# SKA-INAF/caesar-yolo

Measured on AMD Instinct MI355X. Metric: 512x512 tiles/sec over 16k x 16k FITS, higher is better.
Workload: dtype f16

## Files before the change

caesar_yolo_amd/csrc/conv_igemm.hip:

```cpp
#include "cy_kernels.h"
#include <cmath>
#include <cstdlib>
#include <cstring>
#include <vector>

namespace cy {

typedef _Float16 f16;
typedef f16 f16x8 __attribute__((ext_vector_type(8)));
typedef f16 f16x4 __attribute__((ext_vector_type(4)));
typedef float f32x4 __attribute__((ext_vector_type(4)));
typedef unsigned int u32x4 __attribute__((ext_vector_type(4)));
typedef unsigned int u32x2 __attribute__((ext_vector_type(2)));

#define CY_OOB 0xFFFFFF00u
#define CY_WAIT_VM(N) asm volatile("s_waitcnt vmcnt(%0)" ::"n"(N) : "memory")

#ifndef CY_STAMPS_ENABLED
#define CY_STAMPS_ENABLED 0
#endif
__device__ unsigned long long g_stamps[8];
constexpr int WG_STAMP_SLOTS = 4096;
__device__ unsigned long long g_wg_stamps[WG_STAMP_SLOTS * 4];
__device__ __forceinline__ unsigned long long stamp_now() {
// ... 2500 lines not shown
        }
    }
    if (stamps && tid == 0) {
        unsigned long long* rec = g_wg_stamps + (size_t)(blockIdx.x % WG_STAMP_SLOTS) * 4;
        rec[0] = t_loop - t_entry; rec[1] = t_epi - t_loop; rec[2] = stamp_real() - t_epi; rec[3] = c_epi - c_loop;
    }
}

template <int NB, int MI, int RING, bool K3, bool SPLIT = false, int NDW = 8, bool FUSE2 = false>
static hipError_t launch_direct(const ConvArgs& a, hipStream_t s) {
    constexpr int BN = 64 * NB, BM = 8 * MI * 16;
    const size_t lds = (FUSE2 ? 4 : RING) * BN * 128 + 2048;
    static bool attr_set = false;
    if (!attr_set) {
        hipFuncSetAttribute(reinterpret_cast<const void*>(conv1x1_direct_kernel<NB, MI, RING, K3, SPLIT, NDW, FUSE2>), hipFuncAttributeMaxDynamicSharedMemorySize, (int)lds);
        attr_set = true;
    }
    const int M = a.B * a.Ho * a.Wo;
    const int blocks = ((M + BM - 1) / BM) * ((pad64(a.Cout) + BN - 1) / BN);
    hipLaunchKernelGGL((conv1x1_direct_kernel<NB, MI, RING, K3, SPLIT, NDW, FUSE2>), dim3(blocks), dim3(512), lds, s, a);
    return hipGetLastError();
}

template <int WM, int RING>
static hipError_t launch_halo(const ConvArgs& a, hipStream_t s) {
    constexpr int TH = 4 * WM, NT = WM * 128;
    constexpr int PR = (TH + 2) * 18, NWI = (PR + 7) / 8, NW = NT / 64, PROUNDS = (NWI + NW - 1) / NW;
    const size_t lds = 2 * PROUNDS * NW * 1024 + RING * 128 * 128;
    static bool attr_set = false;
    if (!attr_set) {
        hipFuncSetAttribute(reinterpret_cast<const void*>(conv3x3_halo_kernel<WM, RING>), hipFuncAttributeMaxDynamicSharedMemorySize, (int)lds);
        attr_set = true;
    }
    const int blocks = a.B * ((a.Hi + TH - 1) / TH) * ((a.Wi + 15) / 16) * ((pad64(a.Cout) + 127) / 128);
    hipLaunchKernelGGL((conv3x3_halo_kernel<WM, RING>), dim3(blocks), dim3(NT), lds, s, a);
    return hipGetLastError();
}

template <typename T, int WM, int WN, int MI, int NSTAGE = 2, bool SPLIT = false>
static hipError_t launch_t(const ConvArgs& a, hipStream_t s) {
    constexpr int BM = WM * MI * 16, BN = WN * 64;
    const int M = a.B * a.Ho * a.Wo;
    const int ntm = (M + BM - 1) / BM, ntn = (pad64(a.Cout) + BN - 1) / BN;
    const size_t lds = NSTAGE * (BM + BN) * 128;
    static bool attr_set = false;
    if (!attr_set) {
// ... 44 lines not shown
    const size_t lds = head_pair_lds(p, a, b);
    static bool attr_set = false;
    if (!attr_set) {
        hipFuncSetAttribute(reinterpret_cast<const void*>(head1x1_pair_kernel<false>), hipFuncAttributeMaxDynamicSharedMemorySize, 128 * 1024);
        hipFuncSetAttribute(reinterpret_cast<const void*>(head1x1_pair_kernel<true>), hipFuncAttributeMaxDynamicSharedMemorySize, 128 * 1024);
        attr_set = true;
    }
    const long M = (long)a.B * a.Ho * a.Wo;
    const long wgs = (M + 255) / 256;
    const unsigned grid = (unsigned)(wgs < 256 ? wgs : 256);
    if (p == PREC_F16X3) hipLaunchKernelGGL((head1x1_pair_kernel<true>), dim3(grid), dim3(512), lds, s, a, b, head_rows(b), head_pair_pitch(a.out_ct));
    else hipLaunchKernelGGL((head1x1_pair_kernel<false>), dim3(grid), dim3(512), lds, s, a, b, head_rows(b), head_pair_pitch(a.out_ct));
    return hipGetLastError();
}

static const char* const kVariantNames[CONV_NUM_VARIANTS] = {
    "conv_igemm_kernel<2,2,4> generic 128x128", "conv_igemm_kernel<4,1,2> generic 128x64",
    "conv3x3_halo2_kernel 3x3 s1 16x16px x128ch (halo<2,2> for odd slab counts)", "conv3x3_pp_kernel<2> 3x3 s1 16x16px x64ch",
    "conv3x3_c64_kernel<64|32> 3x3 s1 persistent, Cin 64 or 32", "conv_igemm_kernel<4,2,4,3> generic 256x128, 3-slab ring",
    "conv3x3_wide_kernel 3x3 s1 16x32px x128ch, K slabs of 32",
    "conv1x1_direct_kernel<4,2> 1x1 256px x256ch, pixels to regs", "conv1x1_direct_kernel<2,2> 1x1 256px x128ch, pixels to regs",
    "conv3x3_wide_kernel<WN=1> 3x3 s1 16x32px x64ch", "conv3x3_wide_kernel<dual> 3x3 s1 2 images x 16x16px x128ch",
    "conv3x3_widep_kernel<strip> 3x3 s1 512 flattened px x128ch, persistent",
    "head1x1_kernel detect-head output 1x1, weights stationary in LDS, fp32 rows"};
const char* conv_variant_name(int v) { return v >= 0 && v < CONV_NUM_VARIANTS ? kVariantNames[v] : "?"; }

bool batch_invariant() { const char* e = getenv("CY_BATCH_INVARIANT"); return !e || atoi(e) != 0; }

static int conv_variant_x3(const ConvArgs& a) {
    const bool narrow = pad64(a.Cout) <= 64;
    if (a.k == 3 && a.s == 1 && a.c1 == 0 && !a.up0 && !a.out_f32 && a.Cin % 64 == 0 && a.wgt32 && a.out_bs == a.Ho * a.Wo && a.out_ro == 0) {
        const int wpad = (a.Wi + 31) / 32 * 32;
        const bool fits = (wpad - a.Wi) * 8 <= a.Wi;
        if (narrow && a.Wi % 32 == 0) return CONV_WIDE_64;
        if (narrow && a.Cin >= 128 && env_knob("CY_STRIP", 1) && strip_small(a) && strip_fits(a)) return CONV_STRIP_128;
        if (!narrow && env_knob("CY_STRIP", 1) && strip_fits(a) && strip_cover(a.Hi, a.Wi) + 0.04 < wide2d_cover(a.Hi, a.Wi)) return CONV_STRIP_128;
        if (!narrow && fits) return CONV_WIDE_128;
        if (!narrow && a.Wi <= 16 && a.Wi >= 14) return CONV_WIDE_DUAL;
    }
    if (!a.out_f32 && a.Cin % 64 == 0 && !narrow &&
        ((a.k == 1 && a.s == 1 && (a.c1 == 0 || a.c0 % 64 == 0)) || (a.k == 3 && a.s == 2 && a.c1 == 0 && !a.up0)))
        return pad64(a.Cout) >= 256 ? CONV_DIRECT_256 : CONV_DIRECT_128;
    if (head_direct(a, a.split)) return CONV_HEAD_1X1;
    return narrow ? CONV_GENERIC_64 : CONV_GENERIC_128;
}

int conv_variant(Precision p, const ConvArgs& a) {
    if (p == PREC_F16X3) return conv_variant_x3(a);
    const bool narrow = pad64(a.Cout) <= 64;
    const long Bv = batch_invariant() && a.B < 256 ? 256 : a.B;
    if (p == PREC_F16 && a.k == 3 && a.s == 1 && a.c1 == 0 && !a.up0 && !a.out_f32 && a.Cin == 32 && narrow && a.wgt32 &&
        a.out_bs == a.Ho * a.Wo && a.out_ro == 0)
        return CONV_C64_PERSIST;
    if (p == PREC_F16 && a.k == 3 && a.s == 1 && a.c1 == 0 && !a.up0 && !a.out_f32 && a.Cin % 64 == 0 &&
        a.out_bs == a.Ho * a.Wo && a.out_ro == 0) {
        if (narrow && a.wgt32 && a.Cin >= 128 && a.Wi % 32 == 0 && Bv * ((a.Hi + 15) / 16) * (a.Wi / 32) >= 256) return CONV_WIDE_64;
        if (narrow && a.wgt32 && a.Cin >= 128 && env_knob("CY_STRIP", 1) && strip_small(a) && strip_fits(a)) return CONV_STRIP_128;
        if (narrow && a.Cin == 64) return CONV_C64_PERSIST;
        if (narrow) return CONV_PP_64;
        const int strip = env_knob("CY_STRIP", 1);
        if (strip && a.wgt32 && strip_fits(a) && strip_cover(a.Hi, a.Wi) + 0.04 < wide2d_cover(a.Hi, a.Wi) &&
            (strip > 1 || strip_small(a) || Bv * (long)(a.Hi + 1) * (a.Wi + 1) / 512 * ((pad64(a.Cout) + 127) / 128) >= 200))
            return CONV_STRIP_128;
        const int wpad = (a.Wi + 31) / 32 * 32;
        if (a.wgt32 && (wpad - a.Wi) * 8 <= a.Wi) return CONV_WIDE_128;
        const int dual = getenv("CY_WIDE_DUAL") ? atoi(getenv("CY_WIDE_DUAL")) : 1;
        if (dual && a.wgt32 && a.Wi <= 16 && a.Wi >= 14 &&
            ((Bv + 1) / 2) * ((a.Hi + 15) / 16) * ((pad64(a.Cout) + 127) / 128) >= (dual > 1 ? 1 : 224))
            return CONV_WIDE_DUAL;
        return CONV_HALO8_128;
    }
    if (p == PREC_F16 && head_direct(a, 1)) return CONV_HEAD_1X1;
    if (narrow) return CONV_GENERIC_64;
    if (p == PREC_F16 && !a.out_f32 && a.Cin % 64 == 0 &&
        ((a.k == 1 && a.s == 1 && (a.c1 == 0 || a.c0 % 64 == 0)) || (a.k == 3 && a.s == 2 && a.c1 == 0 && !a.up0 && (a.Cin >= 128 || pad64(a.Cout) < 256)))) {
        const char* e = getenv("CY_DIRECT_MIN_BLOCKS");
        const long min_blocks = e ? atol(e) : 256;
        const int bn = pad64(a.Cout) >= 256 ? 256 : 128;
        const long blocks = ((Bv * a.Ho * a.Wo + 255) / 256) * ((pad64(a.Cout) + bn - 1) / bn);
        if (min_blocks >= 0 && blocks >= min_blocks) return bn == 256 ? CONV_DIRECT_256 : CONV_DIRECT_128;
    }
    const long M = Bv * a.Ho * a.Wo;
    if (p == PREC_F16 && (M / 256) * ((pad64(a.Cout) + 127) / 128) >= 256) return CONV_GENERIC_BIG;
    return CONV_GENERIC_128;
}

hipError_t launch_conv(Precision p, const ConvArgs& a, hipStream_t s) {
    if (p == PREC_F16X3) {
        if ((a.split != 2 && a.split != 3) || !a.oscale) return hipErrorInvalidValue;
        switch (conv_variant_x3(a)) {
            case CONV_WIDE_128:
                if (env_knob("CY_X3_PERSIST", 0) && a.Cout % 16 == 0) return launch_widep(a, s);
                return launch_wide<2, false, true>(a, s);
            case CONV_STRIP_128: return launch_strip(a, s);
            case CONV_WIDE_64: return launch_wide<1, false, true>(a, s);
            case CONV_WIDE_DUAL: return launch_wide<2, true, true>(a, s);
            case CONV_DIRECT_256: return a.k == 3 ? launch_direct<4, 2, 3, true, true>(a, s) : launch_direct<4, 2, 3, false, true>(a, s);
            case CONV_DIRECT_128: return a.k == 3 ? launch_direct<2, 4, 2, true, true>(a, s) : launch_direct<2, 2, 2, false, true>(a, s);
            case CONV_HEAD_1X1: return launch_head<true>(a, s);
            case CONV_GENERIC_64: return launch_t<f16, 4, 1, 2, 2, true>(a, s);
            default: return launch_t<f16, 2, 2, 4, 2, true>(a, s);
        }
    }
// ... 4 lines not shown
            ConvArgs b2 = a; b2.dbg = dev_knob("CY_DBG", 0);
            if ((a.Cin / 64) % 2 == 0) return launch_halo2(b2, s);
            return launch_halo<2, 2>(b2, s);
        }
        case CONV_GENERIC_BIG: return launch_t<f16, 4, 2, 4, 3>(a, s);
        case CONV_WIDE_128: {
            ConvArgs b2 = a; b2.dbg = dev_knob("CY_DBG", 0);
            const int wp = env_knob("CY_WIDE_PERSIST", 1);
            const long patches = (long)a.B * ((a.Wi + 31) / 32) * ((a.Hi + 15) / 16) * ((pad64(a.Cout) + 127) / 128);
            if (wp && a.Cout % 16 == 0 && (wp > 1 || (patches >= 512 && a.Cin <= 128))) return launch_widep(b2, s);
            return launch_wide<2>(b2, s);
        }
        case CONV_STRIP_128: return launch_strip(a, s);
        case CONV_WIDE_64: return launch_wide<1>(a, s);
        case CONV_WIDE_DUAL: return launch_wide<2, true>(a, s);
        case CONV_DIRECT_256: {
            ConvArgs a2 = a; a2.dbg = dev_knob("CY_DBG", 0);
            if (a.wgt2 && pad64(a.Cout) == 256 && a.c1 == 0 && !a.res && !a.out_f32)
                return a.k == 3 ? launch_direct<4, 2, 3, true, false, 4, true>(a2, s) : launch_direct<4, 2, 3, false, false, 8, true>(a2, s);
            return a.k == 3 ? launch_direct<4, 2, 3, true, false, 4>(a2, s) : launch_direct<4, 2, 3, false>(a2, s);
        }
        case CONV_DIRECT_128:
            return a.k == 3 ? launch_direct<2, 4, 2, true>(a, s) : launch_direct<2, 2, 2, false>(a, s);
        case CONV_HEAD_1X1: return launch_head<false>(a, s);
        case CONV_GENERIC_64: return p == PREC_F16 ? launch_t<f16, 4, 1, 2>(a, s) : launch_t<float, 4, 1, 2>(a, s);
        default: return p == PREC_F16 ? launch_t<f16, 2, 2, 4>(a, s) : launch_t<float, 2, 2, 4>(a, s);
    }
}

void debug_read_wg_stamps(unsigned long long* out, int n) {
    hipDeviceSynchronize();
    hipMemcpyFromSymbol(out, HIP_SYMBOL(g_wg_stamps), (size_t)(n < WG_STAMP_SLOTS ? n : WG_STAMP_SLOTS) * 4 * sizeof(unsigned long long));
}

void debug_read_stamps(unsigned long long* out8, bool reset) {
    hipDeviceSynchronize();
    hipMemcpyFromSymbol(out8, HIP_SYMBOL(g_stamps), 8 * sizeof(unsigned long long));
    if (CY_STAMPS_ENABLED && out8[6] == 0) {
        static unsigned long long rec[WG_STAMP_SLOTS * 4];
        hipMemcpyFromSymbol(rec, HIP_SYMBOL(g_wg_stamps), sizeof(rec));
        for (int i = 0; i < WG_STAMP_SLOTS; ++i)
            if (rec[i * 4 + 1]) { out8[6] += 1; for (int j = 0; j < 4; ++j) out8[j] += rec[i * 4 + j]; }
        out8[4] = out8[0] + out8[1] + out8[2] + out8[3];
        if (reset) { memset(rec, 0, sizeof(rec)); hipMemcpyToSymbol(HIP_SYMBOL(g_wg_stamps), rec, sizeof(rec)); }
    }
    if (reset) { unsigned long long z[8] = {0}; hipMemcpyToSymbol(HIP_SYMBOL(g_stamps), z, sizeof(z)); }
// ... 761 lines not shown
```

caesar_yolo_amd/csrc/cy_kernels.h:

```cpp
#pragma once
#include <hip/hip_runtime.h>
#include <stdint.h>
#include <stdlib.h>

namespace cy {

#ifndef CY_DEV_KNOBS
#define CY_DEV_KNOBS 0
#endif
inline int env_knob(const char* name, int dflt) { const char* e = getenv(name); return e ? atoi(e) : dflt; }
inline int dev_knob(const char* name, int dflt) { return CY_DEV_KNOBS ? env_knob(name, dflt) : dflt; }

enum Precision { PREC_F16 = 0, PREC_F32 = 1, PREC_F16X3 = 2 };

struct ConvArgs {
    const void* in0; int in0_ct, in0_coff, c0, up0;
    const void* in1; int in1_ct, in1_coff, c1;
    const void* wgt;
    const void* wgt32; uint32_t wgt32_bytes;
    const float* bias;
    void* out; int out_ct, out_coff;
    int out_bs, out_ro;
    int out_f32;
    const void* res; int res_ct, res_coff;
// ... 34 lines not shown
hipError_t launch_bneck64(const BneckArgs& a, hipStream_t s);
void pack_bneck_weights(const float* W1, const float* W2, void* dst);

struct PoolArgs {
    const void* src; void* dst; int ct, src_coff, dst_coff, C, B, H, W;
    int lo;
};

struct DwArgs {
    const void* in; int in_ct, in_coff; void* out; int out_ct, out_coff; const void* res; int res_ct, res_coff;
    const float* w; const float* bias; int B, H, W, C, act;
    int blk, gstride, goff;
    int in_lo, out_lo, res_lo;
    int xcd;
};
struct AttnArgs {
    const void* qkv; int ct, coff; void* out; int out_ct, out_coff; int B, N, heads, kd, hd; float scale;
    int lo, out_lo;
};
hipError_t launch_dwconv(Precision p, const DwArgs& a, hipStream_t s);
hipError_t launch_attention(Precision p, const AttnArgs& a, hipStream_t s);

hipError_t launch_conv(Precision p, const ConvArgs& a, hipStream_t s);
enum ConvVariant { CONV_GENERIC_128 = 0, CONV_GENERIC_64, CONV_HALO8_128, CONV_PP_64, CONV_C64_PERSIST, CONV_GENERIC_BIG, CONV_WIDE_128, CONV_DIRECT_256, CONV_DIRECT_128, CONV_WIDE_64, CONV_WIDE_DUAL, CONV_STRIP_128, CONV_HEAD_1X1, CONV_NUM_VARIANTS };
int conv_variant(Precision p, const ConvArgs& a);
const char* conv_variant_name(int v);
bool head_pair_ok(Precision p, const ConvArgs& a, const ConvArgs& b);
hipError_t launch_head_pair(Precision p, const ConvArgs& a, const ConvArgs& b, hipStream_t s);
void debug_read_stamps(unsigned long long* out8, bool reset);
void debug_read_wg_stamps(unsigned long long* out, int n);
void debug_read_pre_stamps(unsigned long long* out8, bool reset);
void debug_fastdiv(const double* d_a, const double* d_b, double* d_fast, double* d_ref, int n);
hipError_t launch_stem(Precision p, const StemArgs& a, hipStream_t s);
hipError_t launch_stem_down(const StemDownArgs& a, hipStream_t s);
long stem_down_blocks(const StemDownArgs& a);
bool batch_invariant();
void pack_stem_weights2(const float* W, int cout, void* dst);
hipError_t launch_pool5(Precision p, const PoolArgs& a, hipStream_t s);

size_t packed_weight_bytes(Precision p, int cout, int cin, int k, int chunk_bytes = 128);
void pack_weights(Precision p, const float* W, int cout, int cin, int k, void* dst, int chunk_bytes = 128);
void pack_weights_fused2(const float* W2, int cout2, int cin2, void* dst);
int x3_passes(const float* W, int cout, int cin, int k, const float* scale);
size_t packed_weight_bytes_x3(int cout, int cin, int k, int chunk_bytes = 128, int passes = 3);
void pack_weights_x3(const float* W, int cout, int cin, int k, void* dst, float* oscale, int chunk_bytes = 128, int passes = 3, const float* scale = nullptr);
hipError_t launch_x3_split(const float* in, void* out, long npix, int C, hipStream_t s);
hipError_t launch_x3_merge(const void* in, float* out, long npix, int C, hipStream_t s);
// ... 135 lines not shown
```

caesar_yolo_amd/csrc/cy_runtime.hip:

```cpp
#include "../../include/caesar_yolo_hip.h"
#include "cy_kernels.h"
#include "cy_plan.h"
#include <algorithm>
#include <cmath>
#include <cstdio>
#include <cstdlib>
#include <cstring>
#include <string>
#include <vector>

using namespace cy;

struct DevConv { void* w = nullptr; float* bias = nullptr; size_t wbytes = 0; float* stem_w = nullptr; void* w32 = nullptr; size_t w32bytes = 0;
                 float* oscale = nullptr;
                 void* w2f = nullptr; size_t w2fbytes = 0;
                 int passes = 3;
                 float* dw_w = nullptr;
                 void* bneck = nullptr; };

struct cy_ctx {
    int device = 0;
    cy_config cfg{};
    Precision prec = PREC_F16;
    std::string err;
// ... 870 lines not shown
        const Tensor& t = p.tensors[o.out];
        const int Ho = c->lastH >> t.level, Wo = c->lastW >> t.level, C = p.convs[o.conv].cout, B = c->lastB;
        const size_t n = (size_t)B * C * Ho * Wo;
        if (n > cap) return fail(c, CY_ERR_ARG, "output buffer too small");
        HIPCHK(c, hipDeviceSynchronize());
        std::vector<char> host(c->tbytes[o.out]);
        HIPCHK(c, hipMemcpy(host.data(), c->ws + c->toff[o.out], host.size(), hipMemcpyDeviceToHost));
        for (int b = 0; b < B; ++b) for (int h = 0; h < Ho; ++h) for (int w = 0; w < Wo; ++w) for (int ch = 0; ch < C; ++ch) {
            const size_t src = (((size_t)b * Ho + h) * Wo + w) * t.C + o.out_coff + ch;
            float v;
            if (c->prec == PREC_F16X3) {
                const _Float16* hp = reinterpret_cast<_Float16*>(host.data()) + (((size_t)b * Ho + h) * Wo + w) * 2 * t.C + o.out_coff + ch;
                v = (float)hp[0] + (float)hp[t.C];
            } else v = c->prec == PREC_F16 ? (float)reinterpret_cast<_Float16*>(host.data())[src]
                                           : reinterpret_cast<float*>(host.data())[src];
            h_out[(((size_t)b * C + ch) * Ho + h) * Wo + w] = v;
        }
        if (dims4) { dims4[0] = B; dims4[1] = C; dims4[2] = Ho; dims4[3] = Wo; }
        return CY_OK;
    }
    return fail(c, CY_ERR_ARG, std::string("no such conv: ") + conv_name);
}

int cy_conv_bn_silu(cy_ctx* c, const void* d_in, int B, int Hi, int Wi, int Cin, const float* h_w, const float* h_b,
                    int Cout, int k, int s, int act, const void* d_res, void* d_out, void* stream) {
    if (!c || !d_in || !h_w || !h_b || !d_out) return fail(c, CY_ERR_ARG, "null argument");
    if ((k != 1 && k != 3) || (s != 1 && s != 2) || Cin % 8 || B < 1) return fail(c, CY_ERR_ARG, "unsupported conv geometry");
    HIPCHK(c, hipSetDevice(c->device));
    if (c->prec == PREC_F16X3) {
        hipStream_t st = (hipStream_t)stream;
        const int pad = k / 2, Ho = (Hi + 2 * pad - k) / s + 1, Wo = (Wi + 2 * pad - k) / s + 1, cp = (Cout + 127) / 128 * 128;
        const size_t nin = (size_t)B * Hi * Wi, nout = (size_t)B * Ho * Wo;
        const int passes = env_knob("CY_X3_PASSES", 0) == 3 ? 3 : x3_passes(h_w, Cout, Cin, k, nullptr);
        const size_t wb = packed_weight_bytes_x3(Cout, Cin, k, 128, passes), wb32 = (k == 3 && s == 1 && Cin % 64 == 0) ? packed_weight_bytes_x3(Cout, Cin, k, 64, passes) : 0;
        std::vector<char> packed(wb), p32(wb32);
        std::vector<float> osc(cp), bias(cp, 0.0f);
        pack_weights_x3(h_w, Cout, Cin, k, packed.data(), osc.data(), 128, passes);
        if (wb32) pack_weights_x3(h_w, Cout, Cin, k, p32.data(), osc.data(), 64, passes);
        memcpy(bias.data(), h_b, 4 * Cout);
        void *dw = nullptr, *dw32 = nullptr, *xin = nullptr, *xres = nullptr, *xout = nullptr; float *db = nullptr, *dsc = nullptr;
        auto cleanup = [&]() { for (void* q : {dw, dw32, xin, xres, xout, (void*)db, (void*)dsc}) if (q) hipFree(q); };
        hipError_t e = hipMalloc(&dw, wb);
        if (e == hipSuccess && wb32) e = hipMalloc(&dw32, wb32);
        if (e == hipSuccess) e = hipMalloc(&db, 4 * cp);
        if (e == hipSuccess) e = hipMalloc(&dsc, 4 * cp);
        if (e == hipSuccess) e = hipMalloc(&xin, nin * Cin * 4);
// ... 1 lines not shown
        if (e == hipSuccess && d_res) e = hipMalloc(&xres, nout * Cout * 4);
        if (e == hipSuccess) e = hipMemcpy(dw, packed.data(), wb, hipMemcpyHostToDevice);
        if (e == hipSuccess && wb32) e = hipMemcpy(dw32, p32.data(), wb32, hipMemcpyHostToDevice);
        if (e == hipSuccess) e = hipMemcpy(db, bias.data(), 4 * cp, hipMemcpyHostToDevice);
        if (e == hipSuccess) e = hipMemcpy(dsc, osc.data(), 4 * cp, hipMemcpyHostToDevice);
        if (e == hipSuccess) e = launch_x3_split(reinterpret_cast<const float*>(d_in), xin, (long)nin, Cin, st);
        if (e == hipSuccess && d_res) e = launch_x3_split(reinterpret_cast<const float*>(d_res), xres, (long)nout, Cout, st);
        if (e == hipSuccess) {
            ConvArgs a{};
            a.in0 = xin; a.in0_ct = 2 * Cin; a.c0 = Cin; a.in0_bytes = (uint32_t)(nin * Cin * 4); a.in0_lo = Cin;
            a.wgt = dw; a.wgt_bytes = (uint32_t)wb; a.bias = db; a.wgt32 = dw32; a.wgt32_bytes = (uint32_t)wb32; a.oscale = dsc; a.split = passes;
            a.B = B; a.Hi = Hi; a.Wi = Wi; a.Ho = Ho; a.Wo = Wo; a.Cin = Cin; a.Cout = Cout; a.k = k; a.s = s; a.act = act;
            a.out = xout; a.out_ct = 2 * Cout; a.out_lo = Cout; a.out_bs = Ho * Wo;
            if (d_res) { a.res = xres; a.res_ct = 2 * Cout; a.res_lo = Cout; }
            e = launch_conv(c->prec, a, st);
        }
        if (e == hipSuccess) e = launch_x3_merge(xout, reinterpret_cast<float*>(d_out), (long)nout, Cout, st);
        const hipError_t e2 = hipStreamSynchronize(st);
        cleanup();
        if (e != hipSuccess) return fail(c, CY_ERR_HIP, hipGetErrorString(e));
        if (e2 != hipSuccess) return fail(c, CY_ERR_HIP, hipGetErrorString(e2));
        return CY_OK;
    }
    const size_t es = esize(c->prec);
    const size_t wb = packed_weight_bytes(c->prec, Cout, Cin, k);
    std::vector<char> packed(wb);
    pack_weights(c->prec, h_w, Cout, Cin, k, packed.data());
    const int cp = (Cout + 127) / 128 * 128;
    std::vector<float> bias(cp, 0.0f);
    memcpy(bias.data(), h_b, 4 * Cout);
    void* dw = nullptr; float* db = nullptr;
    HIPCHK(c, hipMalloc(&dw, wb));
    HIPCHK(c, hipMalloc(&db, 4 * cp));
    HIPCHK(c, hipMemcpy(dw, packed.data(), wb, hipMemcpyHostToDevice));
    HIPCHK(c, hipMemcpy(db, bias.data(), 4 * cp, hipMemcpyHostToDevice));
    void* dw32 = nullptr; size_t wb32 = 0;
    if (c->prec == PREC_F16 && k == 3 && s == 1 && ((Cin % 64 == 0 && Cout >= 33) || (Cin == 32 && Cout <= 64))) {
        wb32 = packed_weight_bytes(c->prec, Cout, Cin, k, 64);
        std::vector<char> p32(wb32);
        pack_weights(c->prec, h_w, Cout, Cin, k, p32.data(), 64);
        HIPCHK(c, hipMalloc(&dw32, wb32));
        HIPCHK(c, hipMemcpy(dw32, p32.data(), wb32, hipMemcpyHostToDevice));
    }
    ConvArgs a{};
    const int pad = k / 2;
    a.in0 = d_in; a.in0_ct = Cin; a.c0 = Cin; a.in0_bytes = (uint32_t)((size_t)B * Hi * Wi * Cin * es);
    a.wgt = dw; a.wgt_bytes = (uint32_t)wb; a.bias = db; a.wgt32 = dw32; a.wgt32_bytes = (uint32_t)wb32;
    a.B = B; a.Hi = Hi; a.Wi = Wi; a.Ho = (Hi + 2 * pad - k) / s + 1; a.Wo = (Wi + 2 * pad - k) / s + 1;
    a.Cin = Cin; a.Cout = Cout; a.k = k; a.s = s; a.act = act;
    a.out = d_out; a.out_ct = Cout; a.out_bs = a.Ho * a.Wo;
    if (d_res) { a.res = d_res; a.res_ct = Cout; }
    hipError_t e = launch_conv(c->prec, a, (hipStream_t)stream);
    hipError_t e2 = hipStreamSynchronize((hipStream_t)stream);
    hipFree(dw); hipFree(db); if (dw32) hipFree(dw32);
    if (e != hipSuccess) return fail(c, CY_ERR_HIP, hipGetErrorString(e));
    if (e2 != hipSuccess) return fail(c, CY_ERR_HIP, hipGetErrorString(e2));
    return CY_OK;
}

int cy_bottleneck64(cy_ctx* c, const void* d_in, int B, int H, int W, const float* h_w1, const float* h_b1, const float* h_w2,
                    const float* h_b2, int shortcut, void* d_out, void* stream) {
    if (!c || !d_in || !h_w1 || !h_b1 || !h_w2 || !h_b2 || !d_out || B < 1 || H < 1 || W < 1) return fail(c, CY_ERR_ARG, "bad arguments");
    if (c->prec != PREC_F16) return fail(c, CY_ERR_UNSUPPORTED, "the fused bottleneck kernel exists in the fp16 context only");
    HIPCHK(c, hipSetDevice(c->device));
    std::vector<char> wf(BNECK_WFRAG_BYTES);
    pack_bneck_weights(h_w1, h_w2, wf.data());
    void* dw = nullptr; float* db = nullptr;
    HIPCHK(c, hipMalloc(&dw, wf.size()));
    HIPCHK(c, hipMalloc(&db, 128 * sizeof(float)));
    HIPCHK(c, hipMemcpy(dw, wf.data(), wf.size(), hipMemcpyHostToDevice));
    HIPCHK(c, hipMemcpy(db, h_b1, 64 * sizeof(float), hipMemcpyHostToDevice));
    HIPCHK(c, hipMemcpy(db + 64, h_b2, 64 * sizeof(float), hipMemcpyHostToDevice));
    BneckArgs a{};
    a.in = d_in; a.in_ct = 64; a.in_coff = 0; a.in_bytes = (uint32_t)((size_t)B * H * W * 64 * 2);
    a.out = d_out; a.out_ct = 64; a.out_coff = 0; a.wfrag = dw; a.bias1 = db; a.bias2 = db + 64;
    a.B = B; a.H = H; a.W = W; a.shortcut = shortcut != 0;
    hipError_t e = launch_bneck64(a, (hipStream_t)stream);
    hipError_t e2 = hipStreamSynchronize((hipStream_t)stream);
    hipFree(dw); hipFree(db);
    if (e != hipSuccess) return fail(c, CY_ERR_HIP, hipGetErrorString(e));
// ... 748 lines not shown
```

caesar_yolo_amd/lib.py:

```python
import ctypes as C
import os

_HERE = os.path.dirname(os.path.abspath(__file__))
LIB_PATH = os.path.join(_HERE, "libcaesar_yolo_hip.so")

CY_MAX_DET = 300
CY_MAX_STAGES = 8
CY_MEAS_FIELDS = 12
MEAS_NAMES = ("npix", "nring", "bkg", "rms", "peak", "x_peak", "y_peak", "sum", "sw", "swx", "swy", "reserved")
CY_ISL_FIELDS = 20
ISL_NAMES = ("status", "nseed", "nislands", "npix", "npix_main", "nborder", "xmin", "xmax", "ymin", "ymax", "S", "Sx", "Sy", "Sxx", "Syy",
             "Sxy", "S_main", "reserved0", "reserved1", "reserved2")
CY_BKG_FIELDS = 8
BKG_NAMES = ("n0", "n", "bkg", "rms", "L", "H", "rounds", "reserved")
OP_BKG, OP_SHIFT, OP_CLIP, OP_ZSCALE, OP_HISTEQ, OP_MINMAX = 1, 2, 3, 4, 5, 6
F16, F32, F16X3 = 0, 1, 2
PRECISIONS = {"fp16": F16, "f16": F16, "half": F16, "fp32": F32, "f32": F32, "float": F32, "fp16x3": F16X3, "f16x3": F16X3, "split": F16X3}

EXPORTS = [
    "cy_create", "cy_destroy", "cy_last_error", "cy_load_weights", "cy_load_weights_mem", "cy_num_classes",
    "cy_weight_passes", "cy_class_name", "cy_plan_num_convs", "cy_plan_conv_desc", "cy_letterbox_geometry", "cy_num_anchors",
    "cy_pred_elems", "cy_profile_enable", "cy_profile_summary", "cy_profile_summary_lane", "cy_profile_layers", "cy_mosaic_prepare", "cy_letterbox_pack", "cy_preproc", "cy_preproc_planes", "cy_preproc_params", "cy_forward", "cy_debug_read_conv",
    "cy_decode_nms", "cy_debug_stamps", "cy_debug_fastdiv", "cy_debug_cand_counts", "cy_iou_merge", "cy_detect_tiles", "cy_detect_flush", "cy_detect_fence", "cy_compact_records", "cy_compact_records_ctx", "cy_detect_counters", "cy_conv_bn_silu", "cy_bottleneck64", "cy_dwconv3x3",
    "cy_attention", "cy_maxpool5", "cy_make_tile_records",
    "cy_merge_edge_sources", "cy_augment_geometry", "cy_enable_augment", "cy_letterbox_pack_f32", "cy_augment_pack",
    "cy_decode_nms_augmented", "cy_detect_tiles_augmented", "cy_measure_sources", "cy_measure_kernel_ms",
    "cy_measure_islands", "cy_islands_kernel_ms", "cy_measure_background", "cy_background_kernel_ms", "cy_expand_background",
]


class CyError(RuntimeError):
    pass


class cy_config(C.Structure):
    _fields_ = [("precision", C.c_int), ("max_batch", C.c_int), ("max_h", C.c_int), ("max_w", C.c_int),
                ("max_cand", C.c_int)]


class cy_pre_stage(C.Structure):
    _fields_ = [("op", C.c_int), ("p0", C.c_double), ("p1", C.c_double), ("p2", C.c_double), ("flag", C.c_int)]


class cy_pre_program(C.Structure):
    _fields_ = [("n", C.c_int), ("st", cy_pre_stage * CY_MAX_STAGES)]

# ... 60 lines not shown
        "cy_letterbox_pack": (C.c_int, [vp, vp, C.c_int, C.c_int, C.c_int, C.c_int, vp, vp]),
        "cy_forward": (C.c_int, [vp, vp, C.c_int, C.c_int, C.c_int, vp, vp]),
        "cy_profile_enable": (C.c_int, [vp, C.c_int]),
        "cy_profile_summary": (C.c_int, [vp, C.POINTER(cy_prof_entry), C.c_int]),
        "cy_profile_summary_lane": (C.c_int, [vp, C.POINTER(cy_prof_entry), C.c_int, C.c_int]),
        "cy_profile_layers": (C.c_int, [vp, C.POINTER(cy_prof_entry), C.c_int]),
        "cy_debug_read_conv": (C.c_int, [vp, C.c_char_p, fp, C.c_size_t, ip]),
        "cy_decode_nms": (C.c_int, [vp, vp, C.c_int, C.c_int, C.c_int, C.c_int, C.c_int, C.c_float, C.c_float,
                                    vp, vp, vp, vp]),
        "cy_debug_cand_counts": (C.c_int, [vp, ip, C.c_int]),
        "cy_debug_stamps": (C.c_int, [C.POINTER(C.c_ulonglong), C.c_int]),
        "cy_debug_fastdiv": (C.c_int, [vp, vp, vp, vp, C.c_int]),
        "cy_iou_merge": (C.c_int, [vp, vp, vp, C.c_int, C.c_float, C.c_double, C.c_double, vp, vp, vp, vp]),
        "cy_detect_tiles": (C.c_int, [vp, vp, C.c_int, C.c_int, ip, C.c_int, C.c_int, C.c_int, C.c_int,
                                      C.POINTER(cy_preproc_cfg), C.c_float, C.c_float, C.c_double, C.c_double,
                                      vp, vp, vp, vp]),
        "cy_detect_flush": (C.c_int, [vp, vp]),
        "cy_detect_fence": (C.c_int, [vp, vp]),
        "cy_compact_records": (C.c_int, [vp, C.c_longlong, vp, C.c_int, C.c_int, vp, vp, vp]),
        "cy_compact_records_ctx": (C.c_int, [vp, vp, C.c_longlong, vp, C.c_int, C.c_int, vp, vp, vp]),
        "cy_detect_counters": (C.c_int, [vp, C.POINTER(C.c_longlong), C.c_int]),
        "cy_conv_bn_silu": (C.c_int, [vp, vp, C.c_int, C.c_int, C.c_int, C.c_int, fp, fp, C.c_int, C.c_int, C.c_int,
                                      C.c_int, vp, vp, vp]),
        "cy_bottleneck64": (C.c_int, [vp, vp, C.c_int, C.c_int, C.c_int, fp, fp, fp, fp, C.c_int, vp, vp]),
        "cy_dwconv3x3": (C.c_int, [vp, vp, C.c_int, C.c_int, C.c_int, C.c_int, C.c_int, C.c_int, fp, fp, C.c_int, C.c_int, C.c_int,
                                   C.c_int, vp, C.c_int, C.c_int, vp, C.c_int, C.c_int, vp]),
        "cy_attention": (C.c_int, [vp, vp, C.c_int, C.c_int, C.c_int, C.c_int, C.c_int, C.c_int, C.c_int, vp, C.c_int, C.c_int, vp]),
        "cy_maxpool5": (C.c_int, [vp, vp, C.c_int, C.c_int, C.c_int, C.c_int, C.c_int, C.c_int, vp, C.c_int, vp]),
        "cy_make_tile_records": (C.c_int, [fp, ip, C.c_int, ip, C.c_int, dp]),
        "cy_merge_edge_sources": (C.c_int, [dp, C.c_int, ip, C.c_int, dp]),
        "cy_augment_geometry": (C.c_int, [C.c_int, C.c_int, C.POINTER(cy_augment_geom)]),
        "cy_enable_augment": (C.c_int, [vp]),
        "cy_letterbox_pack_f32": (C.c_int, [vp, vp, C.c_int, C.c_int, C.c_int, C.c_int, vp, vp]),
        "cy_augment_pack": (C.c_int, [vp, vp, C.c_int, C.c_int, C.c_int, vp, vp, vp, vp]),
        "cy_decode_nms_augmented": (C.c_int, [vp, vp, vp, vp, C.c_int, C.c_int, C.c_int, C.c_int, C.c_int, C.c_float, C.c_float,
                                              vp, vp, vp, vp]),
        "cy_detect_tiles_augmented": (C.c_int, [vp, vp, C.c_int, C.c_int, ip, C.c_int, C.c_int, C.c_int, C.c_int,
                                                C.POINTER(cy_preproc_cfg), C.c_float, C.c_float, C.c_double, C.c_double, C.c_int,
                                                vp, vp, vp, vp]),
        "cy_measure_sources": (C.c_int, [vp, vp, C.c_int, C.c_int, dp, C.c_int, C.c_int, dp, vp]),
        "cy_measure_kernel_ms": (C.c_int, [vp, dp]),
        "cy_measure_islands": (C.c_int, [vp, vp, C.c_int, C.c_int, dp, dp, C.c_int, C.c_int, dp, vp, C.POINTER(C.c_longlong), vp]),
        "cy_islands_kernel_ms": (C.c_int, [vp, dp]),
        "cy_measure_background": (C.c_int, [vp, vp, C.c_int, C.c_int, C.c_int, C.c_double, C.c_int, dp, vp]),
        "cy_background_kernel_ms": (C.c_int, [vp, dp]),
        "cy_expand_background": (C.c_int, [vp, dp, C.c_int, C.c_int, C.c_int, C.c_int, C.c_int, vp, vp, vp]),
# ... 38 lines not shown
```

caesar_yolo_amd/model.py:

```python
import ctypes as C
import logging
import os
import numpy as np
import torch

from . import lib as L
from . import weights as W


_CPU_WARNED = False


def _dev_index(device):
    if isinstance(device, int):
        return device
    s = str(device)
    if s in ("", "cuda", "gpu"):
        return torch.cuda.current_device()
    if s.startswith("cuda:"):
        return int(s.split(":")[1])
    if s.isdigit():
        return int(s)
    if s == "cpu":
        global _CPU_WARNED
# ... 358 lines not shown

    def bottleneck64(self, x_nhwc, w1, b1, w2, b2, shortcut=True):
        B, H, Wd, Cin = x_nhwc.shape
        out = torch.empty_like(x_nhwc)
        arrs = [np.ascontiguousarray(v, np.float32) for v in (w1, b1, w2, b2)]
        ptr = [v.ctypes.data_as(C.POINTER(C.c_float)) for v in arrs]
        self._chk(self.lib.cy_bottleneck64(self.ctx, self._p(x_nhwc), B, H, Wd, ptr[0], ptr[1], ptr[2], ptr[3], int(bool(shortcut)),
                                           self._p(out), self._stream()))
        return out

    def conv_bn_silu(self, x_nhwc, w, b, k, s, act=True, res=None):
        B, Hi, Wi, Cin = x_nhwc.shape
        Cout = w.shape[0]
        pad = k // 2
        Ho, Wo = (Hi + 2 * pad - k) // s + 1, (Wi + 2 * pad - k) // s + 1
        out = torch.empty((B, Ho, Wo, Cout), dtype=self.dtype, device=self.tdev)
        w = np.ascontiguousarray(w, np.float32)
        b = np.ascontiguousarray(b, np.float32)
        self._chk(self.lib.cy_conv_bn_silu(self.ctx, self._p(x_nhwc), B, Hi, Wi, Cin,
                                           w.ctypes.data_as(C.POINTER(C.c_float)), b.ctypes.data_as(C.POINTER(C.c_float)),
                                           Cout, k, s, int(act), self._p(res) if res is not None else None,
                                           self._p(out), self._stream()))
        return out

    def dwconv3x3(self, x, nch, w, b, out, in_coff=0, out_coff=0, act=True, res=None, res_coff=0, chmap=(0, 0, 0)):
        B, H, Wd, in_ct = x.shape
        w = np.ascontiguousarray(w, np.float32)
        b = np.ascontiguousarray(b, np.float32)
        self._chk(self.lib.cy_dwconv3x3(self.ctx, self._p(x), B, H, Wd, int(nch), in_ct, int(in_coff),
                                        w.ctypes.data_as(C.POINTER(C.c_float)), b.ctypes.data_as(C.POINTER(C.c_float)),
                                        int(bool(act)), int(chmap[0]), int(chmap[1]), int(chmap[2]),
                                        self._p(res) if res is not None else None, res.shape[-1] if res is not None else 0,
                                        int(res_coff), self._p(out), out.shape[-1], int(out_coff), self._stream()))
        return out

    def attention(self, qkv, heads, kd, hd, out, coff=0, out_coff=0):
        B, N, ct = qkv.shape
        self._chk(self.lib.cy_attention(self.ctx, self._p(qkv), B, N, ct, int(coff), int(heads), int(kd), int(hd), self._p(out),
                                        out.shape[-1], int(out_coff), self._stream()))
        return out

    def maxpool5(self, src, nch, dst, src_coff=0, dst_coff=0):
        B, H, Wd, ct = src.shape
        assert tuple(dst.shape) == tuple(src.shape)
        self._chk(self.lib.cy_maxpool5(self.ctx, self._p(src), B, H, Wd, int(nch), ct, int(src_coff), self._p(dst), int(dst_coff),
                                       self._stream()))
# ... 110 lines not shown
```

include/caesar_yolo_hip.h:

```cpp
#ifndef CAESAR_YOLO_HIP_H
#define CAESAR_YOLO_HIP_H
#include <stddef.h>
#include <stdint.h>
#ifdef __cplusplus
extern "C" {
#endif

typedef struct cy_ctx cy_ctx;

enum cy_status { CY_OK = 0, CY_ERR_ARG = -1, CY_ERR_HIP = -2, CY_ERR_IO = -3, CY_ERR_STATE = -4, CY_ERR_UNSUPPORTED = -5 };
enum cy_precision { CY_F16 = 0, CY_F32 = 1, CY_F16X3 = 2 };

#define CY_MAX_DET 300
#define CY_DET_STRIDE 6
#define CY_MAX_STAGES 8
#define CY_MAX_CAND 65535

typedef struct cy_config {
    int precision;
    int max_batch;
    int max_h, max_w;
    int max_cand;
} cy_config;

// ... 53 lines not shown

int cy_debug_stamps(unsigned long long* out8, int reset);
int cy_debug_fastdiv(const double* d_a, const double* d_b, double* d_fast, double* d_ref, int n);
int cy_debug_cand_counts(cy_ctx* ctx, int* h_out, int B);

int cy_iou_merge(cy_ctx* ctx, const float* d_det, const int* d_count, int B, float score_thr, double thr_soft,
                 double thr_hard, float* d_out, int* d_out_count, int* d_out_src, void* stream);

int cy_detect_tiles(cy_ctx* ctx, const float* d_mosaic, int MH, int MW, const int* h_tiles, int B, int th, int tw,
                    int imgsz, const cy_preproc_cfg* cfg, float conf, float iou, double thr_soft, double thr_hard,
                    float* d_out, int* d_out_count, int* d_status, void* stream);

int cy_detect_flush(cy_ctx* ctx, void* stream);
int cy_detect_fence(cy_ctx* ctx, void* stream);

int cy_compact_records(const float* d_gathered, long long n_rows, const long long* d_perm, int T, int row_floats, int* d_hdr, float* d_out, void* stream);
int cy_compact_records_ctx(cy_ctx* ctx, const float* d_gathered, long long n_rows, const long long* d_perm, int T, int row_floats, int* d_hdr, float* d_out, void* stream);

int cy_detect_counters(cy_ctx* ctx, long long* out4, int reset);

int cy_conv_bn_silu(cy_ctx* ctx, const void* d_in, int B, int Hi, int Wi, int Cin, const float* h_w, const float* h_b,
                    int Cout, int k, int s, int act, const void* d_res, void* d_out, void* stream);

int cy_bottleneck64(cy_ctx* ctx, const void* d_in, int B, int H, int W, const float* h_w1, const float* h_b1,
                    const float* h_w2, const float* h_b2, int shortcut, void* d_out, void* stream);

int cy_dwconv3x3(cy_ctx* ctx, const void* d_in, int B, int H, int W, int C, int in_ct, int in_coff, const float* h_w,
                 const float* h_b, int act, int blk, int gstride, int goff, const void* d_res, int res_ct, int res_coff,
                 void* d_out, int out_ct, int out_coff, void* stream);
int cy_attention(cy_ctx* ctx, const void* d_qkv, int B, int N, int ct, int coff, int heads, int kd, int hd, void* d_out,
                 int out_ct, int out_coff, void* stream);
int cy_maxpool5(cy_ctx* ctx, const void* d_src, int B, int H, int W, int C, int ct, int src_coff, void* d_dst, int dst_coff,
                void* stream);

typedef struct cy_augment_view {
    double scale; int flip;
    int ch, cw;
    int Hp, Wp;
    int A;
    int lo, hi;
    int off;
} cy_augment_view;
typedef struct cy_augment_geom { cy_augment_view v[3]; int total; } cy_augment_geom;
int cy_augment_geometry(int H, int W, cy_augment_geom* out);
int cy_enable_augment(cy_ctx* ctx);
int cy_letterbox_pack_f32(cy_ctx* ctx, const double* d_planes, int B, int h0, int w0, int imgsz, float* d_out, void* stream);
// ... 33 lines not shown
```

Baseline: 8958.

## Add weight-stationary persistent 1x1 conv kernel for 128-channel outputs

Adds a persistent 1x1 convolution kernel that loads the full filter and bias into LDS once per workgroup, then loops over pixel groups with a multi-deep register prefetch ring of input loads feeding MFMA. Dispatch sends eligible 1x1 layers with 128 output channels and no residual to it instead of the direct kernel, aiming to remove repeated weight fetches and per-tile launch overhead. It also adds test and introspection APIs for channel-sliced convs and per-layer variant names. The kernel uses up to 128KB of LDS, which limits occupancy to one workgroup per CU, and relies on deep prefetch for latency hiding.

```diff
diff --git a/caesar_yolo_amd/csrc/conv_igemm.hip b/caesar_yolo_amd/csrc/conv_igemm.hip
--- a/caesar_yolo_amd/csrc/conv_igemm.hip
+++ b/caesar_yolo_amd/csrc/conv_igemm.hip
@@ -2546,6 +2546,137 @@
     return hipGetLastError();
 }
 
+template <int NWV, int MI, int D>
+__global__ __launch_bounds__(NWV * 64) void conv1x1_ws_kernel(const ConvArgs a, const int ngrp) {
+    constexpr int NB = 2, PG = 16 * MI, GP = NWV * PG, W_BYTES = NB * 64 * 128;
+    extern __shared__ __attribute__((aligned(16))) char smem[];
+    const int tid = threadIdx.x, lane = tid & 63;
+    const int wave = __builtin_amdgcn_readfirstlane(tid >> 6);
+    const int fr = lane & 15, fq = lane >> 4;
+    const int M = a.B * a.Ho * a.Wo, pch = a.Cin / 64, stride = gridDim.x;
+
+    const auto rsw = __builtin_amdgcn_make_buffer_rsrc(const_cast<void*>(a.wgt), 0, a.wgt_bytes, 0x00020000);
+    const unsigned woff0 = (unsigned)((lane >> 3) * 128 + ((lane & 7) ^ (lane >> 3)) * 16);
+    for (int p = wave; p < pch * (W_BYTES / 1024); p += NWV) dma_piece(rsw, (lds_ptr_t*)(smem + p * 1024), woff0, p * 1024);
+    float* const bias_lds = reinterpret_cast<float*>(smem + pch * W_BYTES);
+    if (wave == 0) {
+        const auto rsb = __builtin_amdgcn_make_buffer_rsrc(const_cast<float*>(a.bias), 0, (unsigned)pad64(a.Cout) * 4u, 0x00020000);
+        dma_piece(rsb, (lds_ptr_t*)bias_lds, lane * 16 < NB * 64 * 4 ? (unsigned)(lane * 16) : CY_OOB, 0);
+    }
+
+    const auto rs0 = __builtin_amdgcn_make_buffer_rsrc(const_cast<void*>(a.in0), 0, a.in0_bytes, 0x00020000);
+    u32x4 x[D][MI][2];
+    int gi = blockIdx.x, vi = 0;
+    unsigned iv[MI];
+    auto group_addr = [&]() {
+        const int m0 = gi < ngrp ? xcd_remap(gi, ngrp) * GP + wave * PG : M;
+#pragma unroll
+        for (int mi = 0; mi < MI; ++mi) {
+            const int m = m0 + mi * 16 + fr;
+            iv[mi] = m < M ? (unsigned)(m * a.in0_ct + a.in0_coff + fq * 8) * 2u : CY_OOB;
+        }
+    };
+    auto issue = [&](u32x4 (&xs)[MI][2]) {
+#pragma unroll
+        for (int mi = 0; mi < MI; ++mi)
+#pragma unroll
+            for (int kk = 0; kk < 2; ++kk) xs[mi][kk] = load_b128(rs0, iv[mi], (vi * 64 + kk * 32) * 2);
+        if (++vi == pch) { vi = 0; gi += stride; group_addr(); }
+    };
+
+    f32x4 acc[NB * 4][MI];
+#pragma unroll
+    for (int ni = 0; ni < NB * 4; ++ni)
+#pragma unroll
+        for (int mi = 0; mi < MI; ++mi) acc[ni][mi] = f32x4{0.f, 0.f, 0.f, 0.f};
+
+    int g = gi, v = 0;
+    auto step = [&](const u32x4 (&xc)[MI][2], u32x4 (&xn)[MI][2]) {
+        issue(xn);
+        const char* Wb = smem + v * W_BYTES;
+        f16x8 wb[2][4];
+        auto load_wb = [&](f16x8* dst, int gq) {
+            const int kk = gq / NB, gb = gq % NB, qf = fq + 4 * kk;
+#pragma unroll
+            for (int ni = 0; ni < 4; ++ni) {
+                const int r = gb * 64 + ni * 16 + fr;
+                dst[ni] = *reinterpret_cast<const f16x8*>(Wb + r * 128 + ((qf ^ (r & 7)) << 4));
+            }
+        };
+        load_wb(wb[0], 0);
+#pragma unroll
+        for (int gq = 0; gq < 2 * NB; ++gq) {
+            const int kk = gq / NB, gb = gq % NB;
+            if (gq + 1 < 2 * NB) load_wb(wb[(gq + 1) & 1], gq + 1);
+#pragma unroll
+            for (int ni = 0; ni < 4; ++ni)
+#pragma unroll
+                for (int mi = 0; mi < MI; ++mi)
+                    acc[gb * 4 + ni][mi] = __builtin_amdgcn_mfma_f32_16x16x32_f16(
+                        wb[gq & 1][ni], __builtin_bit_cast(f16x8, xc[mi][kk]), acc[gb * 4 + ni][mi], 0, 0, 0);
+            __builtin_amdgcn_sched_barrier(0);
+        }
+        if (++v < pch) return;
+        v = 0;
+        const int m0 = g < ngrp ? xcd_remap(g, ngrp) * GP + wave * PG : M;
+#pragma unroll
+        for (int gb = 0; gb < NB; ++gb) {
+            const int cbase = gb * 64 + fq * 16;
+            float bv[16];
+#pragma unroll
+            for (int j = 0; j < 4; ++j) {
+                const f32x4 t = *reinterpret_cast<const f32x4*>(bias_lds + cbase + j * 4);
+                bv[j * 4] = t[0]; bv[j * 4 + 1] = t[1]; bv[j * 4 + 2] = t[2]; bv[j * 4 + 3] = t[3];
+            }
+#pragma unroll
+            for (int mi = 0; mi < MI; ++mi) {
+                const int m = m0 + mi * 16 + fr;
+                float o[16];
+                bias_act16(acc[gb * 4][mi], acc[gb * 4 + 1][mi], acc[gb * 4 + 2][mi], acc[gb * 4 + 3][mi], bv, a.act != 0, o);
+#pragma unroll
+                for (int ni = 0; ni < 4; ++ni) acc[gb * 4 + ni][mi] = f32x4{0.f, 0.f, 0.f, 0.f};
+                if (m >= M || cbase + 16 > a.Cout) continue;
+                f16* dst = reinterpret_cast<f16*>(a.out) + (long)m * a.out_ct + a.out_coff + cbase;
+                f16x8 o0, o1;
+#pragma unroll
+                for (int j = 0; j < 8; ++j) { o0[j] = (f16)o[j]; o1[j] = (f16)o[8 + j]; }
+                *reinterpret_cast<f16x8*>(dst) = o0;
+                *reinterpret_cast<f16x8*>(dst + 8) = o1;
+            }
+        }
+        g += stride;
+    };
+
+    group_addr();
+#pragma unroll
+    for (int d = 0; d < D - 1; ++d) issue(x[d]);
+    CY_WAIT_VM((D - 1) * 2 * MI);
+    __builtin_amdgcn_s_barrier();
+    const int nsteps = ((ngrp - 1 - (int)blockIdx.x) / stride + 1) * pch;
+#pragma unroll 1
+    for (int t = 0; t < nsteps; t += D) {
+#pragma unroll
+        for (int u = 0; u < D; ++u) step(x[u], x[(u + D - 1) % D]);
+    }
+}
+
+template <int NWV, int MI, int D>
+static hipError_t launch_ws_t(const ConvArgs& a, hipStream_t s) {
+    const size_t lds = (size_t)(a.Cin / 64) * 128 * 128 + 1024;
+    static bool attr_set = false;
+    if (!attr_set) {
+        hipFuncSetAttribute(reinterpret_cast<const void*>(conv1x1_ws_kernel<NWV, MI, D>), hipFuncAttributeMaxDynamicSharedMemorySize, 129 * 1024);
+        attr_set = true;
+    }
+    static const int ncu = [] { int dev = 0, n = 256; hipGetDevice(&dev); hipDeviceGetAttribute(&n, hipDeviceAttributeMultiprocessorCount, dev); return n > 0 ? n : 256; }();
+    const long M = (long)a.B * a.Ho * a.Wo;
+    const int ngrp = (int)((M + NWV * 16 * MI - 1) / (NWV * 16 * MI));
+    hipLaunchKernelGGL((conv1x1_ws_kernel<NWV, MI, D>), dim3(ngrp < ncu ? ngrp : ncu), dim3(NWV * 64), lds, s, a, ngrp);
+    return hipGetLastError();
+}
+
+static hipError_t launch_ws(const ConvArgs& a, hipStream_t s) { return launch_ws_t<8, 2, 5>(a, s); }
+
 template <int WM, int RING>
 static hipError_t launch_halo(const ConvArgs& a, hipStream_t s) {
     constexpr int TH = 4 * WM, NT = WM * 128;
@@ -2636,7 +2767,8 @@
     "conv1x1_direct_kernel<4,2> 1x1 256px x256ch, pixels to regs", "conv1x1_direct_kernel<2,2> 1x1 256px x128ch, pixels to regs",
     "conv3x3_wide_kernel<WN=1> 3x3 s1 16x32px x64ch", "conv3x3_wide_kernel<dual> 3x3 s1 2 images x 16x16px x128ch",
     "conv3x3_widep_kernel<strip> 3x3 s1 512 flattened px x128ch, persistent",
-    "head1x1_kernel detect-head output 1x1, weights stationary in LDS, fp32 rows"};
+    "head1x1_kernel detect-head output 1x1, weights stationary in LDS, fp32 rows",
+    "conv1x1_ws_kernel 1x1 x128ch, filter stationary in LDS"};
 const char* conv_variant_name(int v) { return v >= 0 && v < CONV_NUM_VARIANTS ? kVariantNames[v] : "?"; }
 
 bool batch_invariant() { const char* e = getenv("CY_BATCH_INVARIANT"); return !e || atoi(e) != 0; }
@@ -2657,6 +2789,12 @@
         return pad64(a.Cout) >= 256 ? CONV_DIRECT_256 : CONV_DIRECT_128;
     if (head_direct(a, a.split)) return CONV_HEAD_1X1;
     return narrow ? CONV_GENERIC_64 : CONV_GENERIC_128;
+}
+
+static bool ws_fits(const ConvArgs& a) {
+    return a.k == 1 && a.s == 1 && a.c1 == 0 && !a.up0 && a.c0 == a.Cin && !a.out_f32 && !a.res && pad64(a.Cout) == 128 && a.Cout % 16 == 0 && a.Cin % 64 == 0 &&
+           (size_t)a.Cin * 128 * 2 <= 128 * 1024 && a.Ho == a.Hi && a.Wo == a.Wi && a.out_bs == a.Ho * a.Wo && a.out_ro == 0 &&
+           env_knob("CY_PW_STATIONARY", 1);
 }
 
 int conv_variant(Precision p, const ConvArgs& a) {
@@ -2692,7 +2830,7 @@
         const long min_blocks = e ? atol(e) : 256;
         const int bn = pad64(a.Cout) >= 256 ? 256 : 128;
         const long blocks = ((Bv * a.Ho * a.Wo + 255) / 256) * ((pad64(a.Cout) + bn - 1) / bn);
-        if (min_blocks >= 0 && blocks >= min_blocks) return bn == 256 ? CONV_DIRECT_256 : CONV_DIRECT_128;
+        if (min_blocks >= 0 && blocks >= min_blocks) return bn == 256 ? CONV_DIRECT_256 : ws_fits(a) ? CONV_WS_128 : CONV_DIRECT_128;
     }
     const long M = Bv * a.Ho * a.Wo;
     if (p == PREC_F16 && (M / 256) * ((pad64(a.Cout) + 127) / 128) >= 256) return CONV_GENERIC_BIG;
@@ -2743,6 +2881,7 @@
         }
         case CONV_DIRECT_128:
             return a.k == 3 ? launch_direct<2, 4, 2, true>(a, s) : launch_direct<2, 2, 2, false>(a, s);
+        case CONV_WS_128: return launch_ws(a, s);
         case CONV_HEAD_1X1: return launch_head<false>(a, s);
         case CONV_GENERIC_64: return p == PREC_F16 ? launch_t<f16, 4, 1, 2>(a, s) : launch_t<float, 4, 1, 2>(a, s);
         default: return p == PREC_F16 ? launch_t<f16, 2, 2, 4>(a, s) : launch_t<float, 2, 2, 4>(a, s);
diff --git a/caesar_yolo_amd/csrc/cy_kernels.h b/caesar_yolo_amd/csrc/cy_kernels.h
--- a/caesar_yolo_amd/csrc/cy_kernels.h
+++ b/caesar_yolo_amd/csrc/cy_kernels.h
@@ -80,7 +80,7 @@
 hipError_t launch_attention(Precision p, const AttnArgs& a, hipStream_t s);
 
 hipError_t launch_conv(Precision p, const ConvArgs& a, hipStream_t s);
-enum ConvVariant { CONV_GENERIC_128 = 0, CONV_GENERIC_64, CONV_HALO8_128, CONV_PP_64, CONV_C64_PERSIST, CONV_GENERIC_BIG, CONV_WIDE_128, CONV_DIRECT_256, CONV_DIRECT_128, CONV_WIDE_64, CONV_WIDE_DUAL, CONV_STRIP_128, CONV_HEAD_1X1, CONV_NUM_VARIANTS };
+enum ConvVariant { CONV_GENERIC_128 = 0, CONV_GENERIC_64, CONV_HALO8_128, CONV_PP_64, CONV_C64_PERSIST, CONV_GENERIC_BIG, CONV_WIDE_128, CONV_DIRECT_256, CONV_DIRECT_128, CONV_WIDE_64, CONV_WIDE_DUAL, CONV_STRIP_128, CONV_HEAD_1X1, CONV_WS_128, CONV_NUM_VARIANTS };
 int conv_variant(Precision p, const ConvArgs& a);
 const char* conv_variant_name(int v);
 bool head_pair_ok(Precision p, const ConvArgs& a, const ConvArgs& b);
diff --git a/caesar_yolo_amd/csrc/cy_runtime.hip b/caesar_yolo_amd/csrc/cy_runtime.hip
--- a/caesar_yolo_amd/csrc/cy_runtime.hip
+++ b/caesar_yolo_amd/csrc/cy_runtime.hip
@@ -916,6 +916,9 @@
     return fail(c, CY_ERR_ARG, std::string("no such conv: ") + conv_name);
 }
 
+static int conv_layer_slices(cy_ctx* c, const void* d_in, int B, int Hi, int Wi, int Cin, int in_ct, int in_coff, const float* h_w,
+                             const float* h_b, int Cout, int k, int s, int act, const void* d_res, void* d_out, int out_ct, int out_coff,
+                             int* variant, void* stream);
 int cy_conv_bn_silu(cy_ctx* c, const void* d_in, int B, int Hi, int Wi, int Cin, const float* h_w, const float* h_b,
                     int Cout, int k, int s, int act, const void* d_res, void* d_out, void* stream) {
     if (!c || !d_in || !h_w || !h_b || !d_out) return fail(c, CY_ERR_ARG, "null argument");
@@ -963,6 +966,12 @@
         if (e2 != hipSuccess) return fail(c, CY_ERR_HIP, hipGetErrorString(e2));
         return CY_OK;
     }
+    return conv_layer_slices(c, d_in, B, Hi, Wi, Cin, Cin, 0, h_w, h_b, Cout, k, s, act, d_res, d_out, Cout, 0, nullptr, stream);
+}
+
+static int conv_layer_slices(cy_ctx* c, const void* d_in, int B, int Hi, int Wi, int Cin, int in_ct, int in_coff, const float* h_w,
+                             const float* h_b, int Cout, int k, int s, int act, const void* d_res, void* d_out, int out_ct, int out_coff,
+                             int* variant, void* stream) {
     const size_t es = esize(c->prec);
     const size_t wb = packed_weight_bytes(c->prec, Cout, Cin, k);
     std::vector<char> packed(wb);
@@ -985,18 +994,43 @@
     }
     ConvArgs a{};
     const int pad = k / 2;
-    a.in0 = d_in; a.in0_ct = Cin; a.c0 = Cin; a.in0_bytes = (uint32_t)((size_t)B * Hi * Wi * Cin * es);
+    a.in0 = d_in; a.in0_ct = in_ct; a.in0_coff = in_coff; a.c0 = Cin; a.in0_bytes = (uint32_t)((size_t)B * Hi * Wi * in_ct * es);
     a.wgt = dw; a.wgt_bytes = (uint32_t)wb; a.bias = db; a.wgt32 = dw32; a.wgt32_bytes = (uint32_t)wb32;
     a.B = B; a.Hi = Hi; a.Wi = Wi; a.Ho = (Hi + 2 * pad - k) / s + 1; a.Wo = (Wi + 2 * pad - k) / s + 1;
     a.Cin = Cin; a.Cout = Cout; a.k = k; a.s = s; a.act = act;
-    a.out = d_out; a.out_ct = Cout; a.out_bs = a.Ho * a.Wo;
+    a.out = d_out; a.out_ct = out_ct; a.out_coff = out_coff; a.out_bs = a.Ho * a.Wo;
     if (d_res) { a.res = d_res; a.res_ct = Cout; }
+    if (variant) *variant = conv_variant(c->prec, a);
     hipError_t e = launch_conv(c->prec, a, (hipStream_t)stream);
     hipError_t e2 = hipStreamSynchronize((hipStream_t)stream);
     hipFree(dw); hipFree(db); if (dw32) hipFree(dw32);
     if (e != hipSuccess) return fail(c, CY_ERR_HIP, hipGetErrorString(e));
     if (e2 != hipSuccess) return fail(c, CY_ERR_HIP, hipGetErrorString(e2));
     return CY_OK;
+}
+
+int cy_conv_bn_silu_slices(cy_ctx* c, const void* d_in, int B, int Hi, int Wi, int Cin, int in_ct, int in_coff, const float* h_w,
+                           const float* h_b, int Cout, int k, int s, int act, const void* d_res, void* d_out, int out_ct, int out_coff,
+                           int* variant, void* stream) {
+    if (!c || !d_in || !h_w || !h_b || !d_out) return fail(c, CY_ERR_ARG, "null argument");
+    if (c->prec == PREC_F16X3) return fail(c, CY_ERR_UNSUPPORTED, "channel-slice layers: fp16 / fp32 contexts only");
+    if ((k != 1 && k != 3) || (s != 1 && s != 2) || Cin % 8 || in_ct % 8 || in_coff % 8 || out_ct % 8 || out_coff % 8 || B < 1 ||
+        in_coff < 0 || in_coff + Cin > in_ct || out_coff < 0 || out_coff + Cout > out_ct)
+        return fail(c, CY_ERR_ARG, "unsupported conv geometry");
+    HIPCHK(c, hipSetDevice(c->device));
+    return conv_layer_slices(c, d_in, B, Hi, Wi, Cin, in_ct, in_coff, h_w, h_b, Cout, k, s, act, d_res, d_out, out_ct, out_coff, variant, stream);
+}
+
+const char* cy_conv_variant_name(int v) { return conv_variant_name(v); }
+
+int cy_profile_layer_variants(cy_ctx* c, int* out, int cap) {
+    if (!c || !c->loaded || !out) return fail(c, CY_ERR_ARG, "bad arguments");
+    const int n = (int)c->plan.convs.size();
+    if (cap < n) return fail(c, CY_ERR_ARG, "need one entry per conv");
+    for (int i = 0; i < n; ++i) out[i] = -1;
+    for (const auto& r : c->prof)
+        if (r.conv >= 0 && r.conv < n) out[r.conv] = r.kind;
+    return n;
 }
 
 int cy_bottleneck64(cy_ctx* c, const void* d_in, int B, int H, int W, const float* h_w1, const float* h_b1, const float* h_w2,
diff --git a/caesar_yolo_amd/lib.py b/caesar_yolo_amd/lib.py
--- a/caesar_yolo_amd/lib.py
+++ b/caesar_yolo_amd/lib.py
@@ -22,6 +22,7 @@
     "cy_weight_passes", "cy_class_name", "cy_plan_num_convs", "cy_plan_conv_desc", "cy_letterbox_geometry", "cy_num_anchors",
     "cy_pred_elems", "cy_profile_enable", "cy_profile_summary", "cy_profile_summary_lane", "cy_profile_layers", "cy_mosaic_prepare", "cy_letterbox_pack", "cy_preproc", "cy_preproc_planes", "cy_preproc_params", "cy_forward", "cy_debug_read_conv",
     "cy_decode_nms", "cy_debug_stamps", "cy_debug_fastdiv", "cy_debug_cand_counts", "cy_iou_merge", "cy_detect_tiles", "cy_detect_flush", "cy_detect_fence", "cy_compact_records", "cy_compact_records_ctx", "cy_detect_counters", "cy_conv_bn_silu", "cy_bottleneck64", "cy_dwconv3x3",
+    "cy_conv_bn_silu_slices", "cy_conv_variant_name", "cy_profile_layer_variants",
     "cy_attention", "cy_maxpool5", "cy_make_tile_records",
     "cy_merge_edge_sources", "cy_augment_geometry", "cy_enable_augment", "cy_letterbox_pack_f32", "cy_augment_pack",
     "cy_decode_nms_augmented", "cy_detect_tiles_augmented", "cy_measure_sources", "cy_measure_kernel_ms",
@@ -128,6 +129,10 @@
         "cy_detect_counters": (C.c_int, [vp, C.POINTER(C.c_longlong), C.c_int]),
         "cy_conv_bn_silu": (C.c_int, [vp, vp, C.c_int, C.c_int, C.c_int, C.c_int, fp, fp, C.c_int, C.c_int, C.c_int,
                                       C.c_int, vp, vp, vp]),
+        "cy_conv_bn_silu_slices": (C.c_int, [vp, vp, C.c_int, C.c_int, C.c_int, C.c_int, C.c_int, C.c_int, fp, fp, C.c_int, C.c_int, C.c_int,
+                                             C.c_int, vp, vp, C.c_int, C.c_int, C.POINTER(C.c_int), vp]),
+        "cy_conv_variant_name": (C.c_char_p, [C.c_int]),
+        "cy_profile_layer_variants": (C.c_int, [vp, C.POINTER(C.c_int), C.c_int]),
         "cy_bottleneck64": (C.c_int, [vp, vp, C.c_int, C.c_int, C.c_int, fp, fp, fp, fp, C.c_int, vp, vp]),
         "cy_dwconv3x3": (C.c_int, [vp, vp, C.c_int, C.c_int, C.c_int, C.c_int, C.c_int, C.c_int, fp, fp, C.c_int, C.c_int, C.c_int,
                                    C.c_int, vp, C.c_int, C.c_int, vp, C.c_int, C.c_int, vp]),
diff --git a/caesar_yolo_amd/model.py b/caesar_yolo_amd/model.py
--- a/caesar_yolo_amd/model.py
+++ b/caesar_yolo_amd/model.py
@@ -404,6 +404,25 @@
                                            Cout, k, s, int(act), self._p(res) if res is not None else None,
                                            self._p(out), self._stream()))
         return out
+
+    def conv_bn_silu_slices(self, x_nhwc, in_coff, w, b, out, out_coff, act=True, res=None):
+        B, Hi, Wi, in_ct = x_nhwc.shape
+        Cout, Cin, k = w.shape[0], w.shape[1], w.shape[2]
+        w = np.ascontiguousarray(w, np.float32)
+        b = np.ascontiguousarray(b, np.float32)
+        variant = C.c_int(-1)
+        self._chk(self.lib.cy_conv_bn_silu_slices(self.ctx, self._p(x_nhwc), B, Hi, Wi, Cin, in_ct, int(in_coff),
+                                                  w.ctypes.data_as(C.POINTER(C.c_float)), b.ctypes.data_as(C.POINTER(C.c_float)),
+                                                  Cout, k, 1, int(act), self._p(res) if res is not None else None, self._p(out),
+                                                  out.shape[-1], int(out_coff),
+                                                  C.byref(variant), self._stream()))
+        return self.lib.cy_conv_variant_name(variant.value).decode()
+
+    def profile_layer_variants(self):
+        rows = self.profile_layers()
+        kinds = (C.c_int * 256)()
+        n = self._chk(self.lib.cy_profile_layer_variants(self.ctx, kinds, 256))
+        return {rows[i]["name"]: self.lib.cy_conv_variant_name(kinds[i]).decode() for i in range(n) if kinds[i] >= 0}
 
     def dwconv3x3(self, x, nch, w, b, out, in_coff=0, out_coff=0, act=True, res=None, res_coff=0, chmap=(0, 0, 0)):
         B, H, Wd, in_ct = x.shape
diff --git a/include/caesar_yolo_hip.h b/include/caesar_yolo_hip.h
--- a/include/caesar_yolo_hip.h
+++ b/include/caesar_yolo_hip.h
@@ -99,6 +99,12 @@
 int cy_conv_bn_silu(cy_ctx* ctx, const void* d_in, int B, int Hi, int Wi, int Cin, const float* h_w, const float* h_b,
                     int Cout, int k, int s, int act, const void* d_res, void* d_out, void* stream);
 
+int cy_conv_bn_silu_slices(cy_ctx* ctx, const void* d_in, int B, int Hi, int Wi, int Cin, int in_ct, int in_coff, const float* h_w,
+                           const float* h_b, int Cout, int k, int s, int act, const void* d_res, void* d_out, int out_ct, int out_coff,
+                           int* variant, void* stream);
+const char* cy_conv_variant_name(int v);
+int cy_profile_layer_variants(cy_ctx* ctx, int* out, int cap);
+
 int cy_bottleneck64(cy_ctx* ctx, const void* d_in, int B, int H, int W, const float* h_w1, const float* h_b1,
                     const float* h_w2, const float* h_b2, int shortcut, void* d_out, void* stream);
 
```

After: 8983, median of 3. About the same (+0.3%).
